# openhumanoids/pronto

Hardware: AMD Instinct MI355X
Metric: EKF predict+update steps/sec (batched filters), 15-state, 1000 Hz IMU (higher is better)
Workload: dtype f64

## Files before the change

### pronto_amd/csrc/pb_ctx.hpp

```cpp
#pragma once

#include <hip/hip_runtime.h>

#include <algorithm>
#include <cstdarg>
#include <cstdio>
#include <cstdlib>
#include <cstring>
#include <type_traits>
#include <vector>

#include "../../include/pronto_batch.h"
#include "rbis_tile_io.hpp"
#include "rbis_coop.hpp"
#include "rbis_legodo.hpp"
#include "rbis_jointfilt.hpp"
#include "rbis_yawlock.hpp"
#include "rbis_score.hpp"

using namespace pb;

#define PB_MAX_FENCES 16

struct pb_ctx {
// ... 41 lines not shown
  uint8_t *yaw_standing = nullptr;
  double *yaw_gyro = nullptr;
  bool yaw_standing_dev = false, yaw_gyro_dev = false;
  int yaw_standing_all = 0;
  double yaw_gyro_all = 0.0;
  ScorePar score_par;
  double *scored = nullptr;
  int64_t *scorei = nullptr;
  double *notch = nullptr;
  NotchCoef notch_coef;
  bool notch_ready = false;
  double *ins_last = nullptr;
  int64_t *ins_prev_ut = nullptr;
  const uint8_t *imu_valid_next = nullptr;
  const uint8_t *imu_valid_cur = nullptr;
  double *imu_keep = nullptr;
  const uint8_t *imu_idle_cur = nullptr;
  hipEvent_t fence[PB_MAX_FENCES] = {};
  int n_fences = 0;
  hipEvent_t ev_upload = nullptr;
  void *stage = nullptr;
  size_t stage_bytes = 0;
  void *in_stage[2] = { nullptr, nullptr };
  size_t in_stage_bytes[2] = { 0, 0 };
  int in_idx = 0;
  hipStream_t copy_stream = nullptr;
  hipEvent_t ev_consumed[2] = { nullptr, nullptr }, ev_copied = nullptr;
  Consts k{ 9.80665, 1e-6 };
  int64_t utime = 0;
  bool have_state = false;
  bool half15 = false;
  bool replay_onelane = false;
  bool coop15 = false;
  int mem_hint = 0;
  int run_block = 0, run_block_hint = 0;
  bool run_block_coop15 = false;
  bool quad21 = true;
  bool generic_update = false;
  bool smooth_attr = false;
  bool smooth_wide_attr = false;
  int n_cu = 256;
  hipEvent_t ev0 = nullptr, ev1 = nullptr;
  std::vector<void *> owned;
  char err[512] = { 0 };
};

inline thread_local char g_create_err[512] = "";

inline int fail(pb_ctx *c, int code, const char *fmt, ...)
{
  char *dst = c ? c->err : g_create_err;
  va_list ap;
  va_start(ap, fmt);
  vsnprintf(dst, 512, fmt, ap);
  va_end(ap);
  return code;
}

#define HIPCHK(c, call)                                                                               \
  do {                                                                                                \
    hipError_t e_ = (call);                                                                           \
    if (e_ != hipSuccess) return fail((c), PB_ERR_HIP, "%s failed: %s", #call, hipGetErrorString(e_)); \
  } while (0)

inline int nblk(int n) { return (n + 63) / 64; }

// ... 122 lines not shown
    }
    if (what & LEG_TIMES) {
      if (c->leg_ut_on) times.utimes = c->leg_ut_ext ? c->leg_ut_ext : c->leg_ut;
      if (c->leg_valid_on) times.valid = c->leg_valid_ext ? c->leg_valid_ext : c->leg_valid;
      c->leg_ut_on = c->leg_valid_on = false;
      c->leg_ut_ext = nullptr;
      c->leg_valid_ext = nullptr;
    }
    HIPCHK(c, hipSetDevice(c->dev));
    if ((what & (PRED_REFUSE | PRED_FORGET)) && c->pred_slot >= 0) {
      c->pred_slot = -1;
      if (what & PRED_REFUSE)
        return fail(c, PB_ERR_STATE, "%s: no predicted slot here (pb_set_pred_slot is for pb_step_legodo / _split / _correct)", fn);
    }
    if ((what & PRED_WITH_OUT) && c->pred_slot >= 0 && c->out_slot < 0) {
      c->pred_slot = -1;
      return fail(c, PB_ERR_STATE, "%s: no predicted slot here without an output slot (pb_set_output_slot)", fn);
    }
    if ((what & NEEDS_STATE) && !c->have_state) return fail(c, PB_ERR_STATE, "%s before pb_reset", fn);
    if ((what & PRED_TAKE) && c->pred_slot >= 0 && (c->pred_slot >= c->nhist || c->pred_slot == c->out_slot || c->pred_slot == pb_head_slot(c)))
      return fail(c, PB_ERR_ARG, "predicted slot %d: out of range, the output slot or the head's slot", c->pred_slot);
    return PB_OK;
  }
};
#define CALL(c, flags)               \
  Call call((c), __func__, (flags)); \
  if (call.rc) return call.rc

const double *pbk_idle_prepare(pb_ctx *c, const double *imu_dev, StepBcast &bc, int *rc_out);
int pbk_idle_restore(pb_ctx *c, double *out, double *pred, const double q[4]);

int pbk_step(pb_ctx *c, bool update, const double *imu, const double *lo, const uint8_t *mask, const double q[4],
             const StepBcast *bcast = nullptr);
int pbk_step_range(pb_ctx *c, const double *imu, const double *lo, const uint8_t *mask, const double q[4], long b0, int nb, bool coop15, int mem_hint);
int pbk_step_leg(pb_ctx *c, const double *imu, const StepBcast *bcast, const double q[4], const LegIn &lin, int64_t utime, const LegMeasPar &mp,
                 double *lo_out, uint8_t *mask_out);
int pbk_step_leg15(pb_ctx *c, double *out, const double *imu, const double q[4], const StepBcast &bc, const LegIn &lin, const LegStepArgs &la);
int pbk_step_leg21(pb_ctx *c, double *out, const double *imu, const double q[4], const StepBcast &bc, const LegIn &lin, const LegStepArgs &la);
int pbk_legpar15(pb_ctx *c, double *out, const double *imu, const double q[4], const StepBcast &bc, const LegIn &lin, const LegStepArgs &la);
int pbk_legpar21(pb_ctx *c, double *out, const double *imu, const double q[4], const StepBcast &bc, const LegIn &lin, const LegStepArgs &la);
int pbk_replay_fused(pb_ctx *c, int T, const double *imu, const double *lo, const uint8_t *mask, const double q[4], int slot0 = -1);
int pbk_step_pred_kernel(pb_ctx *c, double *out, double *pred, const double *imu, const double *lo, const uint8_t *mask, const double q[4],
                         const StepBcast &bc);
int pbk_step_corr_pred_kernel(pb_ctx *c, int corr_kind, double *out, double *pred, const double *imu, const double *lo, const uint8_t *mask,
                              const double q[4], const CorrArgs &ca, const StepBcast &bc);
int pbk_step_correct(pb_ctx *c, int corr_kind, const double *imu, const double *lo, const uint8_t *mask, const double q[4],
                     const double *z2, const double *r2, const double *rb2, const double *qm2, const uint8_t *mask2,
                     const StepBcast *bcast = nullptr, const double *zb = nullptr, const double *qb = nullptr);
int pbk_update15(pb_ctx *c, int m, const int *idx, const double *z, const double *R, int rkind, const double *rb,
                 const double *qm, const uint8_t *mask);
int pbk_update21(pb_ctx *c, int m, const int *idx, const double *z, const double *R, int rkind, const double *rb,
                 const double *qm, const uint8_t *mask);
int pbk_update21_m123(pb_ctx *c, int m, const int *idx, const double *z, const double *R, int rkind, const double *rb, const double *qm,
                      const uint8_t *mask);
int pbk_update21_m45(pb_ctx *c, int m, const int *idx, const double *z, const double *R, int rkind, const double *rb, const double *qm,
                     const uint8_t *mask);
int pbk_update21_m6(pb_ctx *c, int m, const int *idx, const double *z, const double *R, int rkind, const double *rb, const double *qm,
                    const uint8_t *mask);
int pbk_update_ct(pb_ctx *c, int m, const int *idx, const double *z, const double *r2, const double *rb2, const double *qm,
                  const uint8_t *mask, const double *zb = nullptr, const double *qb = nullptr, const double *rfull = nullptr);
int pbk_smooth_step(pb_ctx *c, const double *next_pred, const double *next_sm, const double *cur, double *out, double dt);
int pbk_smooth_wide(pb_ctx *c, const double *next_pred, const double *next_sm, const double *cur, double *out, double dt);
int pbk_slot_select(pb_ctx *c, double *dst, const double *src, const uint8_t *mask_dev, int when);
int pbk_update_common(pb_ctx *c, int m, const int *idx, const double *z, const double *R, int rkind, const double *qm, bool orient,
                      const uint8_t *mask, int mem);
```

### pronto_amd/csrc/pb_step.hip

```cpp
#include "pb_ctx.hpp"
#include "rbis_step_kernels.hpp"
#include "rbis_replay_kernels.hpp"

template <bool UPDATE, int MH>
static void launch_step_kernel(pb_ctx *c, const double *st, double *out, int nb, bool coop15, bool half, const double *imu, const double *lo,
                               const uint8_t *mask, const double q[4], const StepBcast &bc, const Consts &k)
{
  const int B = c->B;
  if (c->ns == 15 && coop15) {
    Consts kk = k;
    kk.half_tiles = half ? 1 : 0;
    k_step_coop<15, UPDATE, MH><<<nblk(nb) * (half ? 2 : 1), 128, 0, c->stream>>>(st, out, B, imu, lo, mask, q[0], q[1], q[2], q[3], kk, CorrArgs(), bc);
  } else if (c->ns == 15) {
    k_step<15, UPDATE, MH><<<(nb + PB_STEP_BLOCK - 1) / PB_STEP_BLOCK, PB_STEP_BLOCK, 0, c->stream>>>(st, out, B, imu, lo, mask, q[0], q[1], q[2], q[3], k, bc);
  } else if (c->quad21) {
    k_step_quad<UPDATE, MH><<<nblk(nb), 256, 0, c->stream>>>(st, out, B, imu, lo, mask, q[0], q[1], q[2], q[3], k, bc);
  } else {
    k_step_coop<21, UPDATE, MH><<<nblk(nb), 128, 0, c->stream>>>(st, out, B, imu, lo, mask, q[0], q[1], q[2], q[3], k, CorrArgs(), bc);
  }
}

template <bool UPDATE>
static int launch_step(pb_ctx *c, const double *imu, const double *lo, const uint8_t *mask, const double q[4], const StepBcast &bcast)
{
  double *out = update_target(c);
  int rc = PB_OK;
  StepBcast bc = bcast;
  imu = pbk_idle_prepare(c, imu, bc, &rc);
  if (rc) return rc;
  with_mem_hint(c->mem_hint, [&](auto mh) {
    launch_step_kernel<UPDATE, decltype(mh)::value>(c, c->st, out, c->B, c->coop15, c->half15, imu, lo, mask, q, bc, c->k);
  });
  LAUNCHCHK(c);
  if ((rc = pbk_idle_restore(c, out, nullptr, q))) return rc;
  update_done(c, out);
  return PB_OK;
}

int pbk_step_range(pb_ctx *c, const double *imu, const double *lo, const uint8_t *mask, const double q[4], long b0, int nb, bool coop15, int mem_hint)
{
  if (c->st != c->st_base || c->out_slot >= 0 || (c->B & 63) || (b0 & 63) || (nb & 63) || b0 + nb > c->B)
    return fail(c, PB_ERR_STATE, "pbk_step_range: whole tiles of a head that lives in the context's own array");
  const size_t tile_doubles = c->state_doubles / (size_t) (c->stride / 64);
  double *st = c->st + (size_t) (b0 / 64) * tile_doubles;
  const uint8_t *mask_b = mask ? mask + b0 : nullptr;
  Consts kk = c->k;
  if (kk.qblk) kk.qblk += b0;
  with_mem_hint(mem_hint, [&](auto mh) {
    launch_step_kernel<true, decltype(mh)::value>(c, st, st, nb, coop15, false, imu + b0, lo + b0, mask_b, q, StepBcast(), kk);
  });
  LAUNCHCHK(c);
  return PB_OK;
}

static int step_pred(pb_ctx *c, const double *imu, const double *lo, const uint8_t *mask, const double q[4], const StepBcast &bcast)
{
  double *pred = slot_ptr(c, c->pred_slot);
  const int ps = c->pred_slot;
  c->pred_slot = -1;
  int rc = PB_OK;
  StepBcast bc = bcast;
  imu = pbk_idle_prepare(c, imu, bc, &rc);
  if (rc) return rc;
  double *out = update_target(c);
  if (pbk_step_pred_kernel(c, out, pred, imu, lo, mask, q, bc) == PB_OK) {
    LAUNCHCHK(c);
    if ((rc = pbk_idle_restore(c, out, pred, q))) return rc;
    update_done(c, out);
    return PB_OK;
  }
  double *head = c->st;
  const int os = c->out_slot;
  c->out_slot = ps;
  rc = launch_step<false>(c, imu, nullptr, nullptr, q, bc);
  c->st = head;
  c->out_slot = os;
  if (rc) return rc;
  return launch_step<true>(c, imu, lo, mask, q, bc);
}

int pbk_step(pb_ctx *c, bool update, const double *imu, const double *lo, const uint8_t *mask, const double q[4],
             const StepBcast *bcast)
// ... 100 lines not shown
```

### pronto_amd/csrc/pronto_batch.hip

```cpp
#include <algorithm>
#include <new>

#include "pb_ctx.hpp"
#include "rbis_util_kernels.hpp"

#define PB_VERSION_STR "pronto_batch 0.3 gfx950"

extern "C" const char *pb_version(void) { return PB_VERSION_STR; }

extern "C" const char *pb_last_error(const pb_ctx *ctx) { return ctx ? ctx->err : g_create_err; }

extern "C" int pb_create(pb_ctx **out, int n_states, int batch, int device, int n_snapshots)
{
  if (!out) return fail(nullptr, PB_ERR_ARG, "pb_create: out is NULL");
  *out = nullptr;
  if (n_states != 15 && n_states != 21) return fail(nullptr, PB_ERR_ARG, "pb_create: n_states must be 15 or 21");
  if (batch <= 0 || n_snapshots < 0) return fail(nullptr, PB_ERR_ARG, "pb_create: bad batch / n_snapshots");
  int ndev = 0;
  if (hipGetDeviceCount(&ndev) != hipSuccess || ndev <= 0)
    return fail(nullptr, PB_ERR_NO_DEVICE, "pb_create: no HIP device visible (this library has no CPU fallback)");
  if (device < 0 || device >= ndev) return fail(nullptr, PB_ERR_ARG, "pb_create: device %d out of range", device);
  hipDeviceProp_t prop;
  HIPCHK(nullptr, hipGetDeviceProperties(&prop, device));
  if (strncmp(prop.gcnArchName, "gfx950", 6) != 0)
    return fail(nullptr, PB_ERR_NO_DEVICE, "pb_create: device %d is %s; kernels are built for gfx950 only", device,
                prop.gcnArchName);
  pb_ctx *c = new (std::nothrow) pb_ctx();
  if (!c) return fail(nullptr, PB_ERR_ARG, "pb_create: out of host memory");
  c->ns = n_states;
  c->B = batch;
  c->dev = device;
  c->nsnap = n_snapshots;
  c->n_cu = prop.multiProcessorCount > 0 ? prop.multiProcessorCount : 256;
  {
    const char *e = getenv("PRONTO_BATCH_COOP15");
    c->coop15 = e ? (e[0] == '1') : (batch <= 393216);
    const char *eh = getenv("PRONTO_BATCH_HALF");
    c->half15 = c->coop15 && n_states == 15 && eh && eh[0] == '1';
    const char *er = getenv("PRONTO_BATCH_REPLAY_ONELANE");
    c->replay_onelane = er && er[0] == '1';
  }
  c->stride = ((long) batch + 63) / 64 * 64;
  c->nc = (n_states == 15) ? Lay<15>::NC : Lay<21>::NC;
  c->state_doubles = (size_t) c->stride * (size_t) ((n_states == 15) ? Slots<15>::NSLOT : Slots<21>::NSLOT);
  {
    const char *e = getenv("PRONTO_BATCH_XCD");
    c->k.xcd_remap = e ? (e[0] == '1') : 1;
    const long state_bytes = (long) c->state_doubles * 8;
    const char *gu = getenv("PRONTO_BATCH_GENERIC_UPDATE");
    c->generic_update = gu && gu[0] == '1';
    const char *q21 = getenv("PRONTO_BATCH_QUAD21");
    c->quad21 = !(q21 && q21[0] == '0');
    const char *h = getenv("PRONTO_BATCH_MEMHINT");
    c->mem_hint = h ? (h[0] - '0')
                    : (state_bytes < (48L << 20)    ? MH_DEFAULT
                       : state_bytes < (310L << 20) ? MH_STORE_SC1
                       : state_bytes < (350L << 20) ? MH_DEFAULT
                                                    : MH_STREAM_NT);
    if (c->mem_hint < 0 || c->mem_hint > 2) c->mem_hint = MH_DEFAULT;
    {
      const char *eb = getenv("PRONTO_BATCH_BLOCKED"), *ef = getenv("PRONTO_BATCH_BLOCK_FILTERS");
      const long per_filter = state_bytes / c->stride;
      long want = ef ? atol(ef) : (n_states == 15 ? 229376 : 114688);
      want = (want + 63) / 64 * 64;
      const bool on = eb ? (eb[0] == '1') : (state_bytes > (256L << 20));
      if (on && want >= 64 && want < batch && (batch & 63) == 0) {
        const long nblocks = (batch + want - 1) / want;
        c->run_block = (int) (((batch + nblocks - 1) / nblocks + 63) / 64 * 64);
        const long blk_bytes = (long) c->run_block * per_filter;
        c->run_block_hint = h ? c->mem_hint : (blk_bytes < (48L << 20) ? MH_DEFAULT : MH_STORE_SC1);
        const char *e15 = getenv("PRONTO_BATCH_COOP15");
        c->run_block_coop15 = e15 ? (e15[0] == '1') : true;
      }
    }
  }
  if ((unsigned long long) batch * 36ull * 8ull >= (1ull << 32)) {
    delete c;
    return fail(nullptr, PB_ERR_ARG, "pb_create: batch %d too large for one context (input blocks must stay below 4 GiB; "
                "split the batch over several contexts)", batch);
  }
#define CRCHK(call) CRCHK_AS(#call, call)
#define CRCHK_AS(what, call)                                                                        \
  do {                                                                                              \
    hipError_t e_ = (call);                                                                         \
    if (e_ != hipSuccess) {                                                                         \
      fail(nullptr, PB_ERR_HIP, "%s failed: %s", what, hipGetErrorString(e_));                       \
      pb_destroy(c);                                                                                \
      return PB_ERR_HIP;                                                                            \
    }                                                                                               \
  } while (0)
  CRCHK(hipSetDevice(device));
  CRCHK(hipStreamCreateWithFlags(&c->own_stream, hipStreamNonBlocking));
  c->stream = c->own_stream;
  CRCHK_AS("hipMalloc (state)", dev_alloc_hip(c, c->st_base, c->state_doubles));
  c->st = c->st_base;
  CRCHK(hipMemsetAsync(c->st, 0, sizeof(double) * c->state_doubles, c->stream));
  if (n_snapshots > 0) {
    CRCHK_AS("hipMalloc (snapshots)", dev_alloc_hip(c, c->snaps, (size_t) 7 * c->stride * n_snapshots));
    CRCHK(hipMemsetAsync(c->snaps, 0, sizeof(double) * 7 * c->stride * n_snapshots, c->stream));
  }
  CRCHK_AS("hipMalloc (small staging)", dev_alloc_hip(c, c->d_small, 1024));
  CRCHK(hipEventCreate(&c->ev0));
  CRCHK(hipEventCreate(&c->ev1));
  CRCHK(hipStreamCreateWithFlags(&c->copy_stream, hipStreamNonBlocking));
  CRCHK(hipEventCreateWithFlags(&c->ev_consumed[0], hipEventDisableTiming));
// ... 39 lines not shown
{
  if (!c) return PB_ERR_ARG;
  if (c->stream != c->own_stream) HIPCHK(c, hipStreamSynchronize(c->stream));
  c->stream = c->own_stream;
  return PB_OK;
}

extern "C" int pb_set_constants(pb_ctx *c, double g, double chi_tol)
{
  if (!c) return PB_ERR_ARG;
  if (!(g > 0) || !(chi_tol >= 0)) return fail(c, PB_ERR_ARG, "pb_set_constants: g must be > 0 and chi_tol >= 0");
  c->k.g = g;
  c->k.chi_tol = chi_tol;
  return PB_OK;
}

extern "C" int pb_sync(pb_ctx *c)
{
  if (!c) return PB_ERR_ARG;
  HIPCHK(c, hipSetDevice(c->dev));
  HIPCHK(c, hipStreamSynchronize(c->stream));
  return PB_OK;
}

extern "C" int pb_run_block(const pb_ctx *c) { return c ? c->run_block : 0; }

extern "C" const char *pb_hot_kernel(const pb_ctx *c)
{
  if (!c) return "";
  static const char *const names[4][3] = { { "k_step_quad<true,0>", "k_step_quad<true,1>", "k_step_quad<true,2>" },
                                           { "k_step_coop<21,true,0>", "k_step_coop<21,true,1>", "k_step_coop<21,true,2>" },
                                           { "k_step_coop<15,true,0>", "k_step_coop<15,true,1>", "k_step_coop<15,true,2>" },
                                           { "k_step<15,true,0>", "k_step<15,true,1>", "k_step<15,true,2>" } };
  return names[c->ns == 21 ? (c->quad21 ? 0 : 1) : (c->coop15 ? 2 : 3)][c->mem_hint];
}
extern "C" int pb_batch(const pb_ctx *c) { return c ? c->B : -1; }
extern "C" int pb_n_states(const pb_ctx *c) { return c ? c->ns : -1; }

extern "C" int pb_malloc(pb_ctx *c, uint64_t bytes, void **p)
{
  if (!c || !p) return PB_ERR_ARG;
  HIPCHK(c, hipSetDevice(c->dev));
  HIPCHK(c, hipMalloc(p, bytes));
  return PB_OK;
}
extern "C" int pb_free(pb_ctx *c, void *p)
{
  if (!c) return PB_ERR_ARG;
  HIPCHK(c, hipSetDevice(c->dev));
  HIPCHK(c, hipStreamSynchronize(c->stream));
  HIPCHK(c, hipFree(p));
  return PB_OK;
}
extern "C" int pb_memcpy_h2d(pb_ctx *c, void *d, const void *h, uint64_t bytes)
{
  if (!c || (!d && bytes) || (!h && bytes)) return PB_ERR_ARG;
  HIPCHK(c, hipSetDevice(c->dev));
  HIPCHK(c, hipMemcpyAsync(d, h, bytes, hipMemcpyHostToDevice, c->stream));
  HIPCHK(c, hipStreamSynchronize(c->stream));
  return PB_OK;
}
extern "C" int pb_memcpy_d2h(pb_ctx *c, void *h, const void *d, uint64_t bytes)
{
  if (!c || (!d && bytes) || (!h && bytes)) return PB_ERR_ARG;
  HIPCHK(c, hipSetDevice(c->dev));
  HIPCHK(c, hipMemcpyAsync(h, d, bytes, hipMemcpyDeviceToHost, c->stream));
// ... 271 lines not shown
                { z2, sizeof(double) * m2 * B, 0 }, { rbc ? nullptr : R2, rbc ? 0 : sizeof(double) * m2 * B, 0 },
                { quat_meas2, sizeof(double) * 4 * B, 0 }, { mask2, B, 0 } };
  if (mem == PB_HOST_BROADCAST && mem2 == PB_HOST_BROADCAST && rbc && !mask && !mask2 && arg_kernel) {
    StepBcast bc;
    (void) imu_in(c, imu_block, mem, bc, p);
    memcpy(bc.lo, lo_block, sizeof(bc.lo));
    bc.on |= 2;
    return pbk_step_correct(c, corr_kind, nullptr, nullptr, nullptr, q, nullptr, nullptr, R2, nullptr, nullptr, &bc, z2, quat_meas2);
  }
  int rc;
  if (mem == mem2) rc = stage_in(c, mem, p, 7);
  else {
    rc = stage_in(c, mem, p, 3);
    if (!rc) rc = stage_in(c, mem2, p + 3, 4);
  }
  if (rc) return rc;
  return pbk_step_correct(c, corr_kind, (const double *) p[0].dev, (const double *) p[1].dev, (const uint8_t *) p[2].dev, q,
                          (const double *) p[3].dev, (const double *) p[4].dev, rbc ? R2 : nullptr, (const double *) p[5].dev,
                          (const uint8_t *) p[6].dev);
}

extern "C" int pb_run_legodo(pb_ctx *c, int n_steps, const double *imu_stream, const double *lo_stream,
                             const uint8_t *mask_stream, const double q[4], float *elapsed_ms)
{
  CALL(c, PRED_REFUSE | NEEDS_STATE);
  if (n_steps < 0 || !imu_stream || !lo_stream || !q) return fail(c, PB_ERR_ARG, "pb_run_legodo: bad argument");
  const size_t B = (size_t) c->B;
  if (int rc = timed_begin(c, elapsed_ms)) return rc;
  if (c->run_block > 0 && n_steps > 1 && c->st == c->st_base && c->out_slot < 0) {
    for (long b0 = 0; b0 < (long) B; b0 += c->run_block) {
      const int nb = (int) std::min<long>(c->run_block, (long) B - b0);
      for (int s = 0; s < n_steps; s++) {
        int rc = pbk_step_range(c, imu_stream + (size_t) s * 7 * B, lo_stream + (size_t) s * 6 * B,
                                mask_stream ? mask_stream + (size_t) s * B : nullptr, q, b0, nb, c->run_block_coop15, c->run_block_hint);
        if (rc) return rc;
      }
    }
  } else {
    for (int s = 0; s < n_steps; s++) {
      int rc = pbk_step(c, true, imu_stream + (size_t) s * 7 * B, lo_stream + (size_t) s * 6 * B,
                        mask_stream ? mask_stream + (size_t) s * B : nullptr, q);
      if (rc) return rc;
    }
  }
  return timed_end(c, elapsed_ms);
}

static int replay_impl(pb_ctx *c, const char *who, int n_steps, int steps_per_launch, const double *imu_stream, const double *lo_stream,
                       const uint8_t *mask_stream, const double q[4], bool write_through, int first_slot, float *elapsed_ms)
{
  if (n_steps < 0 || steps_per_launch < 1 || !imu_stream || !lo_stream || !q) return fail(c, PB_ERR_ARG, "%s: bad argument", who);
  if (write_through && (first_slot < 0 || first_slot + n_steps > c->nhist))
    return fail(c, PB_ERR_ARG, "%s: slots %d..%d of %d (pb_history_reserve)", who, first_slot, first_slot + n_steps - 1, c->nhist);
  const size_t B = (size_t) c->B;
  if (int rc = detach_head(c, true)) return rc;
  if (int rc = timed_begin(c, elapsed_ms)) return rc;
  for (int s = 0; s < n_steps; s += steps_per_launch) {
    const int T = (n_steps - s < steps_per_launch) ? n_steps - s : steps_per_launch;
    int rc = pbk_replay_fused(c, T, imu_stream + (size_t) s * 7 * B, lo_stream + (size_t) s * 6 * B,
                              mask_stream ? mask_stream + (size_t) s * B : nullptr, q, write_through ? first_slot + s : -1);
    if (rc) return rc;
  }
  return timed_end(c, elapsed_ms);
}

extern "C" int pb_replay_legodo_fused(pb_ctx *c, int n_steps, int steps_per_launch, const double *imu_stream,
                                      const double *lo_stream, const uint8_t *mask_stream, const double q[4],
// ... 382 lines not shown
```

### pronto_amd/csrc/rbis_device.hpp

```cpp
#pragma once

#include <cmath>
#include <type_traits>
#include <utility>

#if defined(__HIPCC__)
#include <hip/hip_runtime.h>
#define PB_HD __host__ __device__ __forceinline__
#else
#define PB_HD inline
#endif

namespace pb {

template <int NS>
struct Lay {
  static constexpr int NB = NS / 3;
  static constexpr int NP = NS * (NS + 1) / 2;
  static constexpr int OFF_VEC = 0;
  static constexpr int OFF_QUAT = NS;
  static constexpr int OFF_LL = NS + 4;
  static constexpr int OFF_P = NS + 5;
  static constexpr int NC = NS + 5 + NP;
};
// ... 9 lines not shown
  return i;
}
PB_HD constexpr int pk_col(int p) { return p - pk_row(p) * (pk_row(p) + 1) / 2; }

template <class Fn, int... I>
PB_HD void static_for_impl(Fn &&fn, std::integer_sequence<int, I...>)
{
  (fn(std::integral_constant<int, I>{}), ...);
}
template <int N, class Fn>
PB_HD void static_for(Fn &&fn)
{
  static_for_impl(fn, std::make_integer_sequence<int, N>{});
}

PB_HD constexpr int core_full(int s) { return s < 9 ? 3 + s : 15 + (s - 9); }
PB_HD constexpr int passive_full(int p) { return p < 3 ? p : 12 + (p - 3); }

template <int NS>
struct Slots {
  using L = Lay<NS>;
  static constexpr bool HB = (NS == 21);
  static constexpr int NSC = HB ? 15 : 9;
  static constexpr int NSB = HB ? 5 : 3;
  static constexpr int NROW = (L::NC + 1) / 2, NSLOT = 2 * NROW;
  static constexpr int TILE = 64;
  static constexpr long TILE_DOUBLES = (long) NSLOT * TILE;
  static constexpr unsigned TILE_BYTES = (unsigned) (NSLOT * TILE * 8);
  struct Tab {
    short slot_of[L::NC];
    short comp_of[NSLOT];
    signed char role2[NSLOT];
    bool split2[NROW];
    int ncore;
    int nq[4];
  };
  static constexpr Tab make()
  {
    Tab t{};
    int s = 0, role = 0;
    auto put = [&](int c) { t.slot_of[c] = (short) s; t.role2[s] = (signed char) role; t.comp_of[s++] = (short) c; };
    if (!HB) {
      for (int i = 0; i < 9; i++) put(L::OFF_VEC + 3 + i);
      for (int i = 0; i < 4; i++) put(L::OFF_QUAT + i);
      for (int i = 0; i < 9; i++)
        for (int j = 0; j <= i; j++) put(L::OFF_P + pk(core_full(i), core_full(j)));
      t.ncore = s;
      t.nq[0] = t.nq[1] = s;
      role = 1;
      for (int J = 0; J < 2; J++)
        for (int i = 0; i < NSC; i++)
          for (int cc = 0; cc < 3; cc++) put(L::OFF_P + pk(core_full(i), passive_full(3 * J + cc)));
      for (int i = 0; i < 6; i++)
        for (int j = 0; j <= i; j++) put(L::OFF_P + pk(passive_full(i), passive_full(j)));
      put(L::OFF_LL);
      for (int i = 0; i < 6; i++) put(L::OFF_VEC + passive_full(i));
      t.nq[2] = s;
    } else {
      for (int i = 0; i < 9; i++)
        for (int j = 0; j <= i; j++) put(L::OFF_P + pk(core_full(i), core_full(j)));
      put(L::OFF_LL);
      t.nq[0] = s;
      for (int i = 9; i < NSC; i++)
        for (int j = 0; j <= i; j++) put(L::OFF_P + pk(core_full(i), core_full(j)));
      for (int i = 0; i < 6; i++) put(L::OFF_VEC + 15 + i);
      role = 1;
      for (int i = 0; i < 3; i++) put(L::OFF_VEC + passive_full(i));
      t.nq[1] = s;
      t.ncore = s;
      for (int i = 0; i < NSC; i++)
        for (int cc = 0; cc < 3; cc++) put(L::OFF_P + pk(core_full(i), passive_full(cc)));
      for (int i = 0; i < 3; i++)
        for (int j = 0; j <= i; j++) put(L::OFF_P + pk(passive_full(i), passive_full(j)));
      role = 0;
      for (int i = 0; i < 9; i++) put(L::OFF_VEC + 3 + i);
      for (int i = 0; i < 4; i++) put(L::OFF_QUAT + i);
      t.nq[2] = s;
      role = 1;
      for (int i = 0; i < NSC; i++)
        for (int cc = 0; cc < 3; cc++) put(L::OFF_P + pk(core_full(i), passive_full(3 + cc)));
      for (int i = 3; i < 6; i++)
        for (int j = 0; j <= i; j++) put(L::OFF_P + pk(passive_full(i), passive_full(j)));
      for (int i = 3; i < 6; i++) put(L::OFF_VEC + passive_full(i));
    }
    while (s < NSLOT) { t.role2[s] = (signed char) role; t.comp_of[s++] = -1; }
    t.nq[3] = s;
    for (int r = 0; r < NROW; r++) t.split2[r] = t.role2[2 * r] != t.role2[2 * r + 1];
    return t;
  }
  static constexpr Tab T = make();
  static_assert(T.nq[0] % 2 == 0 && T.nq[1] % 2 == 0 && T.nq[2] % 2 == 0, "every wave must own whole rows");
  static constexpr int ROW_SPLIT = T.ncore / 2;
  static constexpr int QROW[5] = { 0, T.nq[0] / 2, T.nq[1] / 2, T.nq[2] / 2, T.nq[3] / 2 };
  PB_HD static constexpr int slot(int comp) { return T.slot_of[comp]; }
  PB_HD static long eidx(int comp, long b)
  {
    const int sl = T.slot_of[comp];
    return (b >> 6) * TILE_DOUBLES + (long) (sl >> 1) * (2 * TILE) + (b & 63) * 2 + (sl & 1);
  }
  PB_HD static long eidx_slot(int sl, long b) { return (b >> 6) * TILE_DOUBLES + (long) (sl >> 1) * (2 * TILE) + (b & 63) * 2 + (sl & 1); }
};

enum { BW = 0, BV = 1, BCHI = 2, BPOS = 3, BACC = 4, BBG = 5, BBA = 6 };

struct Consts {
  double g;
  double chi_tol;
  const double *qblk = nullptr;
  int xcd_remap = 0;
  int half_tiles = 0;
};

PB_HD void quat_mul(const double (&a)[4], const double (&b)[4], double (&o)[4])
{
  const double w = a[0] * b[0] - a[1] * b[1] - a[2] * b[2] - a[3] * b[3];
  const double x = a[0] * b[1] + a[1] * b[0] + a[2] * b[3] - a[3] * b[2];
  const double y = a[0] * b[2] + a[2] * b[0] + a[3] * b[1] - a[1] * b[3];
  const double z = a[0] * b[3] + a[3] * b[0] + a[1] * b[2] - a[2] * b[1];
  o[0] = w; o[1] = x; o[2] = y; o[3] = z;
}
// ... 440 lines not shown
```

### pronto_amd/csrc/rbis_step_kernels.hpp

```cpp
#pragma once

#include "rbis_tile_io.hpp"
#include "rbis_coop.hpp"
#include "rbis_quad.hpp"

namespace pb {

template <int NS, bool UPDATE, int MH = MH_DEFAULT>
__global__ __launch_bounds__(PB_STEP_BLOCK, 1) void k_step(const double *st, double *sto, int B,
                                                const double *__restrict__ imu, const double *__restrict__ lo,
                                                const uint8_t *__restrict__ mask, double qg, double qa, double qbg,
                                                double qba, Consts k, StepBcast bc)
{
  using L = Lay<NS>;
  const unsigned tile = xcd_workgroup(k);
  const unsigned b = tile * 64u + threadIdx.x;
  if (b >= (unsigned) B) return;
  const unsigned bo = b * 8u, B8 = (unsigned) B * 8u;
  TileIO<NS, MemHint<MH>::LA, MemHint<MH>::SA> io(st, sto, tile, threadIdx.x);
  const rsrc_t ri = mkbuf(imu, 7u * B8);
  const rsrc_t rl = mkbuf(lo, UPDATE ? 6u * B8 : 0u);
  double gyro[3], accel[3], dt, z[3], rd[3];
  bool upd = false;
  if constexpr (UPDATE) upd = (mask == nullptr) || (mask[b] != 0);
  if (bc.on & 1) {
#pragma unroll
    for (int i = 0; i < 3; i++) { gyro[i] = bc.imu[i]; accel[i] = bc.imu[3 + i]; }
    dt = bc.imu[6];
  } else {
#pragma unroll
    for (int i = 0; i < 3; i++) {
      gyro[i] = ldg(ri, i * B8, bo);
      accel[i] = ldg(ri, (3 + i) * B8, bo);
    }
    dt = ldg(ri, 6u * B8, bo);
  }
// ... 93 lines not shown
    const rsrc_t rr = mkbuf(ca.r2, ca.r2 ? (unsigned) CORR::M * B8 : 0u);
    const rsrc_t rq2 = mkbuf(ca.qm2, CORR::ORIENT ? 4u * B8 : 0u);
#pragma unroll
    for (int i = 0; i < CORR::M; i++) {
      cin.z[i] = ca.zbc ? ca.zb2[i] : ldg(rz, i * B8, bo);
      cin.rd[i] = ca.r2 ? ldg(rr, i * B8, bo) : ca.rb2[i];
    }
    if (ca.rfull != nullptr) {
      const rsrc_t rf = mkbuf(ca.rfull, (unsigned) (CORR::M * CORR::M) * B8);
#pragma unroll
      for (int i = 0; i < CORR::M; i++) {
        cin.rd[i] = ldg(rf, (unsigned) (i * CORR::M + i) * B8, bo);
#pragma unroll
        for (int j = 0; j < i; j++) cin.ro[i * (i - 1) / 2 + j] = ldg(rf, (unsigned) (j * CORR::M + i) * B8, bo);
      }
    }
#pragma unroll
    for (int i = 0; i < 4; i++) cin.qm[i] = CORR::ORIENT ? (ca.zbc ? ca.qb2[i] : ldg(rq2, i * B8, bo)) : 0.0;
    cin.upd = (b < (unsigned) B) && (ca.mask2 == nullptr || ca.mask2[b] != 0);
    if constexpr (!PREDICT && !UPDATE) {
      if (st == sto && ca.mask2 != nullptr && __ballot(cin.upd) == 0ull) return;
    }
  }
  auto ld = [&io](int comp) { return io.ld(comp); };
  auto stf = [&io](int comp, double v) { io.st(comp, v); };
  auto sync = []() { __syncthreads(); };
  auto xrd = [lane](int s) { return xch[s][lane]; };
  if (role == 0) {
    io.template need<0, Slots<NS>::ROW_SPLIT>();
    coop_role_core<NS, UPDATE, CORR, PREDICT>(ld, stf, [lane](int s, double v) { xch[s][lane] = v; }, xrd, sync, in, k, cin);
  } else {
    io.template need<Slots<NS>::ROW_SPLIT, Slots<NS>::NROW>();
    coop_role_passive<NS, UPDATE, CORR, PREDICT>(ld, stf, xrd, sync, in, k, cin);
  }
}

template <class IO>
struct PredStore {
  static constexpr bool on = true;
  IO *io;
  __device__ __forceinline__ void operator()(int comp, double v) const { io->st(comp, v); }
};

template <int NS, int MH = MH_DEFAULT>
__global__ __launch_bounds__(128, 1) void k_step_coop_pred(const double *st, double *sto, double *pred, int B,
                                                           const double *__restrict__ imu, const double *__restrict__ lo,
                                                           const uint8_t *__restrict__ mask, double qg, double qa,
                                                           double qbg, double qba, Consts k, StepBcast bc)
{
  __shared__ double xch[CoopX<NS, NoCorr>::NXCH][64];
  const int role = __builtin_amdgcn_readfirstlane((int) (threadIdx.x >> 6));
  const unsigned wgi = xcd_workgroup(k);
  const unsigned tile = k.half_tiles ? (wgi >> 1) : wgi;
  const unsigned lane = k.half_tiles ? ((threadIdx.x & 31u) | ((wgi & 1u) << 5)) : (threadIdx.x & 63u);
  const unsigned b = tile * 64u + lane;
  const unsigned bo = b * 8u, B8 = (unsigned) B * 8u;
  using IO = TileIO<NS, MemHint<MH>::LA, MemHint<MH>::SA, true>;
  IO io(st, sto, tile, lane);
  IO po(pred, pred, tile, lane);
  const rsrc_t ri = mkbuf(imu, 7u * B8);
  const rsrc_t rl = mkbuf(lo, 6u * B8);
  StepInputs in;
  if (bc.on & 1) {
#pragma unroll
    for (int i = 0; i < 3; i++) { in.gyro[i] = bc.imu[i]; in.accel[i] = bc.imu[3 + i]; }
    in.dt = bc.imu[6];
// ... 252 lines not shown
```

### pronto_amd/csrc/rbis_tile_io.hpp

```cpp
#pragma once

#include <hip/hip_runtime.h>
#include <stdint.h>

#include "rbis_device.hpp"

#define PB_STEP_BLOCK 64

namespace pb {

typedef unsigned v2u __attribute__((ext_vector_type(2)));
typedef unsigned v4u __attribute__((ext_vector_type(4)));
typedef double d2_t __attribute__((ext_vector_type(2)));
typedef __amdgpu_buffer_rsrc_t rsrc_t;

__device__ __forceinline__ rsrc_t mkbuf(const void *p, unsigned bytes)
{
  return __builtin_amdgcn_make_buffer_rsrc(const_cast<void *>(p), 0, bytes, 0x00020000);
}
template <int AUX = 0>
__device__ __forceinline__ double ldg(rsrc_t r, unsigned soff, unsigned voff)
{
  return __builtin_bit_cast(double, __builtin_amdgcn_raw_buffer_load_b64(r, voff, soff, AUX));
}
// ... 1 lines not shown
__device__ __forceinline__ void stg(rsrc_t r, unsigned soff, unsigned voff, double v)
{
  __builtin_amdgcn_raw_buffer_store_b64(__builtin_bit_cast(v2u, v), r, voff, soff, AUX);
}
template <int AUX = 0>
__device__ __forceinline__ d2_t ldg2(rsrc_t r, unsigned soff, unsigned voff)
{
  return __builtin_bit_cast(d2_t, __builtin_amdgcn_raw_buffer_load_b128(r, voff, soff, AUX));
}
template <int AUX = 0>
__device__ __forceinline__ void stg2(rsrc_t r, unsigned soff, unsigned voff, d2_t v)
{
  const v4u d = __builtin_bit_cast(v4u, v);
  __builtin_amdgcn_raw_buffer_store_b128(d, r, voff, soff, AUX);
  asm volatile("s_nop 1" ::"v"(d));
}

enum { MH_DEFAULT = 0, MH_STORE_SC1 = 1, MH_STREAM_NT = 2 };
template <int MH> struct MemHint {
  static constexpr int LA = (MH == MH_STREAM_NT) ? 2 : 0;
  static constexpr int SA = (MH == MH_STORE_SC1) ? 16 : (MH == MH_STREAM_NT) ? 2 : 0;
};

__device__ __forceinline__ unsigned xcd_workgroup(const Consts &k)
{
  unsigned wg = blockIdx.x;
  if (k.xcd_remap) {
    const unsigned nq = gridDim.x >> 3, nr = gridDim.x & 7u, xcd = blockIdx.x & 7u, rank = blockIdx.x >> 3;
    wg = (xcd < nr ? xcd * (nq + 1u) : nr * (nq + 1u) + (xcd - nr) * nq) + rank;
  }
  return wg;
}

template <int NS, int LA, int SA, bool TWO_ROLE = false>
struct TileIO {
  using S = Slots<NS>;
  rsrc_t rs, ro;
  unsigned vo;
  d2_t cache[S::NROW];
  bool loaded[S::NROW];
  double outv[S::NSLOT];
  bool have[S::NSLOT];
  __device__ __forceinline__ TileIO(const double *st, double *sto, unsigned tile, unsigned lane)
  {
    rs = mkbuf(reinterpret_cast<const char *>(st) + (size_t) tile * S::TILE_BYTES, S::TILE_BYTES);
    ro = mkbuf(reinterpret_cast<char *>(sto) + (size_t) tile * S::TILE_BYTES, S::TILE_BYTES);
    vo = lane * 16u;
#pragma unroll
    for (int r = 0; r < S::NROW; r++) loaded[r] = false;
#pragma unroll
    for (int s = 0; s < S::NSLOT; s++) {
      have[s] = S::T.comp_of[s] < 0;
      outv[s] = 0.0;
    }
  }
  __device__ __forceinline__ void fetch(int r)
  {
    if (!loaded[r]) {
      cache[r] = ldg2<LA>(rs, (unsigned) r * 1024u, vo);
      loaded[r] = true;
    }
  }
  template <int R0, int R1>
  __device__ __forceinline__ void need()
  {
#pragma unroll
    for (int r = R0; r < R1; r++) fetch(r);
  }
  __device__ __forceinline__ double ld(int comp)
  {
    const int s = S::T.slot_of[comp];
    fetch(s >> 1);
    return (s & 1) ? cache[s >> 1].y : cache[s >> 1].x;
  }
  __device__ __forceinline__ void st(int comp, double v)
  {
    const int s = S::T.slot_of[comp];
    if (TWO_ROLE && S::T.split2[s >> 1]) {
      stg<SA>(ro, (unsigned) (s >> 1) * 1024u + (unsigned) (s & 1) * 8u, vo, v);
      return;
    }
    outv[s] = v;
    have[s] = true;
    if (have[s ^ 1]) {
      const d2_t o = { outv[s & ~1], outv[s | 1] };
      stg2<SA>(ro, (unsigned) (s >> 1) * 1024u, vo, o);
    }
  }
  __device__ __forceinline__ double ld_slot_rt(int slot) const
  {
    return ldg(rs, (unsigned) (slot >> 1) * 1024u + (unsigned) (slot & 1) * 8u, vo);
  }
};

template <int NS>
__device__ __forceinline__ int slot_rt(int comp)
{
  return Slots<NS>::T.slot_of[comp];
}
__device__ __forceinline__ int pk_rt(int i, int j) { return i >= j ? i * (i + 1) / 2 + j : j * (j + 1) / 2 + i; }

struct IdxVel {
  static constexpr Idx<3> value = { { 3, 4, 5 } };
};

template <int M>
struct IdxArg {
  int v[M];
};
template <int M>
struct DiagArg {
// ... 31 lines not shown
```

Measured before the change: 2.756 billion.

## Add balanced two-role 15-state step kernel splitting covariance work between wavefronts

Adds k_step_bal15, a two-wavefront cooperative kernel for the 15-state filter. One wave owns the 9x9 core covariance block and computes the 3x3 innovation factorization and gain rows. The other wave propagates the cross and bias blocks plus the state, exchanging values through LDS with one barrier. The aim is to balance work between the two roles better than the existing coop kernel. It is enabled by default only for specific batch-size ranges and adds a new store-split table, which costs extra code complexity and LDS traffic.

```diff
diff --git a/pronto_amd/csrc/pb_ctx.hpp b/pronto_amd/csrc/pb_ctx.hpp
--- a/pronto_amd/csrc/pb_ctx.hpp
+++ b/pronto_amd/csrc/pb_ctx.hpp
@@ -97,6 +97,7 @@
   bool half15 = false;
   bool replay_onelane = false;
   bool coop15 = false;
+  bool bal15 = false, run_block_bal15 = false;
   int mem_hint = 0;
   int run_block = 0, run_block_hint = 0;
   bool run_block_coop15 = false;
@@ -285,7 +286,8 @@
 
 int pbk_step(pb_ctx *c, bool update, const double *imu, const double *lo, const uint8_t *mask, const double q[4],
              const StepBcast *bcast = nullptr);
-int pbk_step_range(pb_ctx *c, const double *imu, const double *lo, const uint8_t *mask, const double q[4], long b0, int nb, bool coop15, int mem_hint);
+int pbk_step_range(pb_ctx *c, const double *imu, const double *lo, const uint8_t *mask, const double q[4], long b0, int nb, bool coop15, bool bal15,
+                   int mem_hint);
 int pbk_step_leg(pb_ctx *c, const double *imu, const StepBcast *bcast, const double q[4], const LegIn &lin, int64_t utime, const LegMeasPar &mp,
                  double *lo_out, uint8_t *mask_out);
 int pbk_step_leg15(pb_ctx *c, double *out, const double *imu, const double q[4], const StepBcast &bc, const LegIn &lin, const LegStepArgs &la);
diff --git a/pronto_amd/csrc/pb_step.hip b/pronto_amd/csrc/pb_step.hip
--- a/pronto_amd/csrc/pb_step.hip
+++ b/pronto_amd/csrc/pb_step.hip
@@ -3,11 +3,13 @@
 #include "rbis_replay_kernels.hpp"
 
 template <bool UPDATE, int MH>
-static void launch_step_kernel(pb_ctx *c, const double *st, double *out, int nb, bool coop15, bool half, const double *imu, const double *lo,
+static void launch_step_kernel(pb_ctx *c, const double *st, double *out, int nb, bool coop15, bool half, bool bal15, const double *imu, const double *lo,
                                const uint8_t *mask, const double q[4], const StepBcast &bc, const Consts &k)
 {
   const int B = c->B;
-  if (c->ns == 15 && coop15) {
+  if (UPDATE && c->ns == 15 && coop15 && bal15 && !half) {
+    k_step_bal15<true, MH><<<nblk(nb), 128, 0, c->stream>>>(st, out, B, imu, lo, mask, q[0], q[1], q[2], q[3], k, bc);
+  } else if (c->ns == 15 && coop15) {
     Consts kk = k;
     kk.half_tiles = half ? 1 : 0;
     k_step_coop<15, UPDATE, MH><<<nblk(nb) * (half ? 2 : 1), 128, 0, c->stream>>>(st, out, B, imu, lo, mask, q[0], q[1], q[2], q[3], kk, CorrArgs(), bc);
@@ -29,7 +31,7 @@
   imu = pbk_idle_prepare(c, imu, bc, &rc);
   if (rc) return rc;
   with_mem_hint(c->mem_hint, [&](auto mh) {
-    launch_step_kernel<UPDATE, decltype(mh)::value>(c, c->st, out, c->B, c->coop15, c->half15, imu, lo, mask, q, bc, c->k);
+    launch_step_kernel<UPDATE, decltype(mh)::value>(c, c->st, out, c->B, c->coop15, c->half15, c->bal15, imu, lo, mask, q, bc, c->k);
   });
   LAUNCHCHK(c);
   if ((rc = pbk_idle_restore(c, out, nullptr, q))) return rc;
@@ -37,7 +39,8 @@
   return PB_OK;
 }
 
-int pbk_step_range(pb_ctx *c, const double *imu, const double *lo, const uint8_t *mask, const double q[4], long b0, int nb, bool coop15, int mem_hint)
+int pbk_step_range(pb_ctx *c, const double *imu, const double *lo, const uint8_t *mask, const double q[4], long b0, int nb, bool coop15, bool bal15,
+                   int mem_hint)
 {
   if (c->st != c->st_base || c->out_slot >= 0 || (c->B & 63) || (b0 & 63) || (nb & 63) || b0 + nb > c->B)
     return fail(c, PB_ERR_STATE, "pbk_step_range: whole tiles of a head that lives in the context's own array");
@@ -47,7 +50,7 @@
   Consts kk = c->k;
   if (kk.qblk) kk.qblk += b0;
   with_mem_hint(mem_hint, [&](auto mh) {
-    launch_step_kernel<true, decltype(mh)::value>(c, st, st, nb, coop15, false, imu + b0, lo + b0, mask_b, q, StepBcast(), kk);
+    launch_step_kernel<true, decltype(mh)::value>(c, st, st, nb, coop15, false, bal15, imu + b0, lo + b0, mask_b, q, StepBcast(), kk);
   });
   LAUNCHCHK(c);
   return PB_OK;
diff --git a/pronto_amd/csrc/pronto_batch.hip b/pronto_amd/csrc/pronto_batch.hip
--- a/pronto_amd/csrc/pronto_batch.hip
+++ b/pronto_amd/csrc/pronto_batch.hip
@@ -9,6 +9,8 @@
 extern "C" const char *pb_version(void) { return PB_VERSION_STR; }
 
 extern "C" const char *pb_last_error(const pb_ctx *ctx) { return ctx ? ctx->err : g_create_err; }
+
+static bool bal15_default(long n) { return (n >= 32768 && n <= 49152) || (n >= 98304 && n <= 131072) || n == 393216; }
 
 extern "C" int pb_create(pb_ctx **out, int n_states, int batch, int device, int n_snapshots)
 {
@@ -37,6 +39,8 @@
     c->coop15 = e ? (e[0] == '1') : (batch <= 393216);
     const char *eh = getenv("PRONTO_BATCH_HALF");
     c->half15 = c->coop15 && n_states == 15 && eh && eh[0] == '1';
+    const char *eb = getenv("PRONTO_BATCH_BAL15");
+    c->bal15 = n_states == 15 && c->coop15 && !c->half15 && (eb ? (eb[0] == '1') : bal15_default(batch));
     const char *er = getenv("PRONTO_BATCH_REPLAY_ONELANE");
     c->replay_onelane = er && er[0] == '1';
   }
@@ -71,6 +75,8 @@
         c->run_block_hint = h ? c->mem_hint : (blk_bytes < (48L << 20) ? MH_DEFAULT : MH_STORE_SC1);
         const char *e15 = getenv("PRONTO_BATCH_COOP15");
         c->run_block_coop15 = e15 ? (e15[0] == '1') : true;
+        const char *eb15 = getenv("PRONTO_BATCH_BAL15");
+        c->run_block_bal15 = n_states == 15 && c->run_block_coop15 && (eb15 ? (eb15[0] == '1') : bal15_default(c->run_block));
       }
     }
   }
@@ -176,6 +182,8 @@
                                            { "k_step_coop<21,true,0>", "k_step_coop<21,true,1>", "k_step_coop<21,true,2>" },
                                            { "k_step_coop<15,true,0>", "k_step_coop<15,true,1>", "k_step_coop<15,true,2>" },
                                            { "k_step<15,true,0>", "k_step<15,true,1>", "k_step<15,true,2>" } };
+  static const char *const bal[3] = { "k_step_bal15<true,0>", "k_step_bal15<true,1>", "k_step_bal15<true,2>" };
+  if (c->ns == 15 && c->coop15 && c->bal15) return bal[c->mem_hint];
   return names[c->ns == 21 ? (c->quad21 ? 0 : 1) : (c->coop15 ? 2 : 3)][c->mem_hint];
 }
 extern "C" int pb_batch(const pb_ctx *c) { return c ? c->B : -1; }
@@ -513,7 +521,8 @@
       const int nb = (int) std::min<long>(c->run_block, (long) B - b0);
       for (int s = 0; s < n_steps; s++) {
         int rc = pbk_step_range(c, imu_stream + (size_t) s * 7 * B, lo_stream + (size_t) s * 6 * B,
-                                mask_stream ? mask_stream + (size_t) s * B : nullptr, q, b0, nb, c->run_block_coop15, c->run_block_hint);
+                                mask_stream ? mask_stream + (size_t) s * B : nullptr, q, b0, nb, c->run_block_coop15, c->run_block_bal15,
+                                c->run_block_hint);
         if (rc) return rc;
       }
     }
diff --git a/pronto_amd/csrc/rbis_coop_bal.hpp b/pronto_amd/csrc/rbis_coop_bal.hpp
--- /dev/null
+++ b/pronto_amd/csrc/rbis_coop_bal.hpp
@@ -0,0 +1,290 @@
+#pragma once
+
+#include "rbis_coop.hpp"
+
+namespace pb {
+
+struct Bal15 {
+  static constexpr int NS = 15, NSC = 9, NPC = 45;
+  static constexpr int X_L = 0, X_ID = 3, X_W = 6, X_NL = 6 + 3 * NSC;
+  static constexpr int NXCH = X_NL + 1;
+};
+
+template <bool UPDATE, class LD, class ST, class XW, class SYNC>
+PB_HD void bal15_role_core(LD ld, ST st, XW xw, SYNC sync, const StepInputs &in, const Consts &k)
+{
+  constexpr int NS = Bal15::NS, NSC = Bal15::NSC;
+  using L = Lay<NS>;
+  using C = Coop<NS>;
+  double x[NS], q[4];
+#pragma unroll
+  for (int i = 0; i < NS; i++) x[i] = ld(L::OFF_VEC + i);
+#pragma unroll
+  for (int i = 0; i < 4; i++) q[i] = ld(L::OFF_QUAT + i);
+  double Pc[Bal15::NPC];
+#pragma unroll
+  for (int i = 0; i < NSC; i++)
+#pragma unroll
+    for (int j = 0; j <= i; j++) Pc[pk(i, j)] = ld(L::OFF_P + pk(C::fullc(i), C::fullc(j)));
+
+  ProcBlocks f;
+  make_proc_blocks<NS>(x, q, in.dt, k, f);
+  if constexpr (!UPDATE) sync();
+  {
+    const int src[2] = { 0, 1 };
+    const int kind[2] = { 0, 0 };
+    double A[2][9];
+#pragma unroll
+    for (int i = 0; i < 9; i++) { A[0][i] = f.A_R[i]; A[1][i] = f.A_RV[i]; }
+    RowOp<NSC, 2, 2>::apply(Pc, src, kind, A);
+  }
+  {
+    const int src[2] = { 0, 1 };
+    const int kind[2] = { 1, 1 };
+    double A[2][9];
+#pragma unroll
+    for (int i = 0; i < 9; i++) { A[0][i] = f.a_mw[i % 3]; A[1][i] = f.a_g[i % 3]; }
+    RowOp<NSC, 0, 2>::apply(Pc, src, kind, A);
+    const int src2[1] = { 1 };
+    const int kind2[1] = { 1 };
+    double A2[1][9];
+#pragma unroll
+    for (int i = 0; i < 9; i++) A2[0][i] = f.a_mw[i % 3];
+    RowOp<NSC, 1, 1>::apply(Pc, src2, kind2, A2);
+  }
+  {
+    const double qgd = in.qg * in.dt, qad = in.qa * in.dt;
+    const double vv = f.v[0] * f.v[0] + f.v[1] * f.v[1] + f.v[2] * f.v[2];
+#pragma unroll
+    for (int r = 0; r < 3; r++)
+#pragma unroll
+      for (int c = 0; c <= r; c++) Pc[pk(r, c)] += qgd * ((r == c ? vv : 0.0) - f.v[r] * f.v[c]) + (r == c ? qad : 0.0);
+    const double m[9] = { 0, f.v[2], -f.v[1], -f.v[2], 0, f.v[0], f.v[1], -f.v[0], 0 };
+#pragma unroll
+    for (int r = 0; r < 3; r++)
+#pragma unroll
+      for (int c = 0; c < 3; c++)
+        if (r != c) Pc[pk(3 + r, c)] += qgd * m[3 * r + c];
+#pragma unroll
+    for (int r = 0; r < 3; r++) Pc[pk(3 + r, 3 + r)] += qgd;
+  }
+  if constexpr (!UPDATE) {
+#pragma unroll
+    for (int i = 0; i < NSC; i++)
+#pragma unroll
+      for (int j = 0; j <= i; j++) st(L::OFF_P + pk(C::fullc(i), C::fullc(j)), Pc[pk(i, j)]);
+  } else {
+    double S[6], d[3], id[3];
+#pragma unroll
+    for (int i = 0; i < 3; i++)
+#pragma unroll
+      for (int j = 0; j <= i; j++) S[pk(i, j)] = Pc[pk(i, j)] + (i == j ? (in.upd ? in.rd[i] : 1.0) : 0.0);
+    ldlt<3>(S, d);
+    double det = 1.0;
+#pragma unroll
+    for (int kk = 0; kk < 3; kk++) {
+      id[kk] = in.upd ? 1.0 / d[kk] : 0.0;
+      det *= d[kk];
+    }
+    const double nl = -log(det);
+    double W[NSC][3];
+#pragma unroll
+    for (int i = 0; i < NSC; i++)
+#pragma unroll
+      for (int kk = 0; kk < 3; kk++) {
+        double s = Pc[pk(i, kk)];
+#pragma unroll
+        for (int j = 0; j < kk; j++) s -= W[i][j] * S[pk(kk, j)];
+        W[i][kk] = s;
+      }
+    xw(Bal15::X_L, S[pk(1, 0)]); xw(Bal15::X_L + 1, S[pk(2, 0)]); xw(Bal15::X_L + 2, S[pk(2, 1)]);
+#pragma unroll
+    for (int kk = 0; kk < 3; kk++) xw(Bal15::X_ID + kk, id[kk]);
+#pragma unroll
+    for (int i = 0; i < NSC; i++)
+#pragma unroll
+      for (int kk = 0; kk < 3; kk++) xw(Bal15::X_W + 3 * i + kk, W[i][kk]);
+    xw(Bal15::X_NL, nl);
+    sync();
+#pragma unroll
+    for (int i = 0; i < NSC; i++) {
+      double wd[3];
+#pragma unroll
+      for (int kk = 0; kk < 3; kk++) wd[kk] = W[i][kk] * id[kk];
+#pragma unroll
+      for (int j = 0; j <= i; j++) {
+        double acc = Pc[pk(i, j)];
+#pragma unroll
+        for (int kk = 0; kk < 3; kk++) acc = fma(-wd[kk], W[j][kk], acc);
+        st(L::OFF_P + pk(C::fullc(i), C::fullc(j)), acc);
+      }
+    }
+  }
+}
+
+template <bool UPDATE, class LD, class ST, class XR, class SYNC>
+PB_HD void bal15_role_passive(LD ld, ST st, XR xr, SYNC sync, const StepInputs &in, const Consts &k)
+{
+  constexpr int NS = Bal15::NS, NSC = Bal15::NSC;
+  using L = Lay<NS>;
+  using C = Coop<NS>;
+  double x[NS], q[4];
+#pragma unroll
+  for (int i = 0; i < NS; i++) x[i] = ld(L::OFF_VEC + i);
+#pragma unroll
+  for (int i = 0; i < 4; i++) q[i] = ld(L::OFF_QUAT + i);
+  double X[3][2][9];
+#pragma unroll
+  for (int sb = 0; sb < 3; sb++)
+#pragma unroll
+    for (int J = 0; J < 2; J++)
+#pragma unroll
+      for (int r = 0; r < 3; r++)
+#pragma unroll
+        for (int c = 0; c < 3; c++) X[sb][J][3 * r + c] = ld(L::OFF_P + pk(C::fullc(3 * sb + r), C::fullp(3 * J + c)));
+  double Ppp[21];
+#pragma unroll
+  for (int i = 0; i < 6; i++)
+#pragma unroll
+    for (int j = 0; j <= i; j++) Ppp[pk(i, j)] = ld(L::OFF_P + pk(C::fullp(i), C::fullp(j)));
+  double ll = ld(L::OFF_LL);
+
+  double xp[6];
+  {
+    ProcBlocks f;
+    make_proc_blocks<NS>(x, q, in.dt, k, f);
+#pragma unroll
+    for (int J = 0; J < 2; J++) {
+      double nD[9], nV[9], nC[9];
+#pragma unroll
+      for (int i = 0; i < 9; i++) { nD[i] = X[2][J][i]; nV[i] = X[0][J][i]; nC[i] = X[1][J][i]; }
+      mat_mul_acc(f.A_R, X[0][J], nD);
+      mat_mul_acc(f.A_RV, X[1][J], nD);
+      hat_mul_acc(f.a_mw, X[0][J], nV);
+      hat_mul_acc(f.a_g, X[1][J], nV);
+      hat_mul_acc(f.a_mw, X[1][J], nC);
+#pragma unroll
+      for (int i = 0; i < 9; i++) { X[2][J][i] = nD[i]; X[0][J][i] = nV[i]; X[1][J][i] = nC[i]; }
+    }
+  }
+#pragma unroll
+  for (int r = 0; r < 3; r++)
+#pragma unroll
+    for (int c = 0; c <= r; c++) {
+      Ppp[pk(r, c)] = (r == c) ? in.qg : 0.0;
+      Ppp[pk(3 + r, 3 + c)] = (r == c) ? in.qa : 0.0;
+    }
+#pragma unroll
+  for (int i = 0; i < 3; i++) {
+    xp[i] = in.gyro[i] - 0.0;
+    xp[3 + i] = in.accel[i] - 0.0;
+  }
+#pragma unroll
+  for (int i = 0; i < 4; i++) pb_pin(q[i]);
+#pragma unroll
+  for (int sb = 0; sb < 3; sb++)
+#pragma unroll
+    for (int J = 0; J < 2; J++)
+#pragma unroll
+      for (int i = 0; i < 9; i++) pb_pin(X[sb][J][i]);
+#pragma unroll
+  for (int i = 0; i < 9; i++) pb_pin(x[C::fullc(i)]);
+  ins_update_state<NS>(x, q, in.gyro, in.accel, in.dt, k);
+#pragma unroll
+  for (int i = 0; i < 9; i++) pb_pin(x[C::fullc(i)]);
+#pragma unroll
+  for (int i = 0; i < 4; i++) pb_pin(q[i]);
+  sync();
+  if constexpr (UPDATE) {
+    const double L10 = xr(Bal15::X_L), L20 = xr(Bal15::X_L + 1), L21 = xr(Bal15::X_L + 2);
+    const double Ls[6] = { 0.0, L10, 0.0, L20, L21, 0.0 };
+    double id[3], resid[3], y[3], yd[3];
+#pragma unroll
+    for (int kk = 0; kk < 3; kk++) id[kk] = xr(Bal15::X_ID + kk);
+#pragma unroll
+    for (int i = 0; i < 3; i++) resid[i] = in.upd ? in.z[i] - x[3 + i] : 0.0;
+    double quad = 0.0;
+#pragma unroll
+    for (int kk = 0; kk < 3; kk++) {
+      double s = resid[kk];
+#pragma unroll
+      for (int j = 0; j < kk; j++) s -= Ls[pk(kk, j)] * y[j];
+      y[kk] = in.upd ? s : 0.0;
+      yd[kk] = y[kk] * id[kk];
+      quad += s * s * id[kk];
+    }
+    const double lli = xr(Bal15::X_NL) - quad;
+    if (in.upd) ll += lli;
+    double Wp[6][3];
+#pragma unroll
+    for (int pi = 0; pi < 6; pi++) {
+      const double c0 = X[0][pi / 3][0 * 3 + pi % 3], c1 = X[0][pi / 3][1 * 3 + pi % 3], c2 = X[0][pi / 3][2 * 3 + pi % 3];
+      Wp[pi][0] = c0;
+      Wp[pi][1] = c1 - Wp[pi][0] * L10;
+      Wp[pi][2] = c2 - Wp[pi][0] * L20 - Wp[pi][1] * L21;
+      xp[pi] += fma(Wp[pi][2], yd[2], fma(Wp[pi][1], yd[1], Wp[pi][0] * yd[0]));
+    }
+#pragma unroll
+    for (int J = 0; J < 2; J++)
+#pragma unroll
+      for (int sb = 0; sb < 3; sb++)
+#pragma unroll
+        for (int r = 0; r < 3; r++) {
+          double wd[3];
+#pragma unroll
+          for (int kk = 0; kk < 3; kk++) wd[kk] = xr(Bal15::X_W + 3 * (3 * sb + r) + kk) * id[kk];
+#pragma unroll
+          for (int c = 0; c < 3; c++) {
+            double acc = X[sb][J][3 * r + c];
+#pragma unroll
+            for (int kk = 0; kk < 3; kk++) acc = fma(-wd[kk], Wp[3 * J + c][kk], acc);
+            st(L::OFF_P + pk(C::fullc(3 * sb + r), C::fullp(3 * J + c)), acc);
+          }
+        }
+#pragma unroll
+    for (int i = 0; i < 6; i++) {
+      double wd[3];
+#pragma unroll
+      for (int kk = 0; kk < 3; kk++) wd[kk] = Wp[i][kk] * id[kk];
+#pragma unroll
+      for (int j = 0; j <= i; j++) {
+        double acc = Ppp[pk(i, j)];
+#pragma unroll
+        for (int kk = 0; kk < 3; kk++) acc = fma(-wd[kk], Wp[j][kk], acc);
+        st(L::OFF_P + pk(C::fullp(i), C::fullp(j)), acc);
+      }
+    }
+    reload_fence();
+    double dfull[NS];
+#pragma unroll
+    for (int i = 0; i < NS; i++) dfull[i] = 0.0;
+#pragma unroll
+    for (int i = 0; i < NSC; i++) {
+      const double w0 = xr(Bal15::X_W + 3 * i), w1 = xr(Bal15::X_W + 3 * i + 1), w2 = xr(Bal15::X_W + 3 * i + 2);
+      dfull[C::fullc(i)] = fma(w2, yd[2], fma(w1, yd[1], w0 * yd[0])) + 0.0;
+    }
+    if (in.upd) add_delta<NS>(x, q, dfull, k.chi_tol);
+  } else {
+#pragma unroll
+    for (int J = 0; J < 2; J++)
+#pragma unroll
+      for (int sb = 0; sb < 3; sb++)
+#pragma unroll
+        for (int r = 0; r < 3; r++)
+#pragma unroll
+          for (int c = 0; c < 3; c++) st(L::OFF_P + pk(C::fullc(3 * sb + r), C::fullp(3 * J + c)), X[sb][J][3 * r + c]);
+#pragma unroll
+    for (int i = 0; i < 6; i++)
+#pragma unroll
+      for (int j = 0; j <= i; j++) st(L::OFF_P + pk(C::fullp(i), C::fullp(j)), Ppp[pk(i, j)]);
+  }
+  st(L::OFF_LL, ll);
+#pragma unroll
+  for (int i = 0; i < 6; i++) st(L::OFF_VEC + C::fullp(i), xp[i]);
+#pragma unroll
+  for (int i = 0; i < 9; i++) st(L::OFF_VEC + C::fullc(i), x[C::fullc(i)]);
+#pragma unroll
+  for (int i = 0; i < 4; i++) st(L::OFF_QUAT + i, q[i]);
+}
+
+}
diff --git a/pronto_amd/csrc/rbis_device.hpp b/pronto_amd/csrc/rbis_device.hpp
--- a/pronto_amd/csrc/rbis_device.hpp
+++ b/pronto_amd/csrc/rbis_device.hpp
@@ -65,6 +65,8 @@
     short comp_of[NSLOT];
     signed char role2[NSLOT];
     bool split2[NROW];
+    signed char role2b[NSLOT];
+    bool split2b[NROW];
     int ncore;
     int nq[4];
   };
@@ -119,6 +121,11 @@
     while (s < NSLOT) { t.role2[s] = (signed char) role; t.comp_of[s++] = -1; }
     t.nq[3] = s;
     for (int r = 0; r < NROW; r++) t.split2[r] = t.role2[2 * r] != t.role2[2 * r + 1];
+    for (int sl = 0; sl < NSLOT; sl++) {
+      const int c = t.comp_of[sl];
+      t.role2b[sl] = HB ? t.role2[sl] : (signed char) ((c >= L::OFF_P && sl < t.ncore) ? 0 : 1);
+    }
+    for (int r = 0; r < NROW; r++) t.split2b[r] = t.role2b[2 * r] != t.role2b[2 * r + 1];
     return t;
   }
   static constexpr Tab T = make();
diff --git a/pronto_amd/csrc/rbis_step_kernels.hpp b/pronto_amd/csrc/rbis_step_kernels.hpp
--- a/pronto_amd/csrc/rbis_step_kernels.hpp
+++ b/pronto_amd/csrc/rbis_step_kernels.hpp
@@ -2,6 +2,7 @@
 
 #include "rbis_tile_io.hpp"
 #include "rbis_coop.hpp"
+#include "rbis_coop_bal.hpp"
 #include "rbis_quad.hpp"
 
 namespace pb {
@@ -161,6 +162,68 @@
   } else {
     io.template need<Slots<NS>::ROW_SPLIT, Slots<NS>::NROW>();
     coop_role_passive<NS, UPDATE, CORR, PREDICT>(ld, stf, xrd, sync, in, k, cin);
+  }
+}
+
+template <bool UPDATE, int MH = MH_DEFAULT>
+__global__ __launch_bounds__(128, 1) void k_step_bal15(const double *st, double *sto, int B,
+                                                       const double *__restrict__ imu, const double *__restrict__ lo,
+                                                       const uint8_t *__restrict__ mask, double qg, double qa,
+                                                       double qbg, double qba, Consts k, StepBcast bc)
+{
+  constexpr int NS = 15;
+  __shared__ double xch[UPDATE ? Bal15::NXCH : 1][64];
+  const int role = __builtin_amdgcn_readfirstlane((int) (threadIdx.x >> 6));
+  const unsigned tile = xcd_workgroup(k);
+  const unsigned lane = threadIdx.x & 63u;
+  const unsigned b = tile * 64u + lane;
+  const unsigned bo = b * 8u, B8 = (unsigned) B * 8u;
+  TileIO<NS, MemHint<MH>::LA, MemHint<MH>::SA, 2> io(st, sto, tile, lane);
+  auto inputs = [&](bool core) {
+    const rsrc_t ri = mkbuf(imu, 7u * B8);
+    const rsrc_t rl = mkbuf(lo, UPDATE ? 6u * B8 : 0u);
+    StepInputs in;
+    if (bc.on & 1) {
+#pragma unroll
+      for (int i = 0; i < 3; i++) { in.gyro[i] = bc.imu[i]; in.accel[i] = bc.imu[3 + i]; }
+      in.dt = bc.imu[6];
+    } else {
+#pragma unroll
+      for (int i = 0; i < 3; i++) {
+        in.gyro[i] = core ? 0.0 : ldg(ri, i * B8, bo);
+        in.accel[i] = core ? 0.0 : ldg(ri, (3 + i) * B8, bo);
+      }
+      in.dt = ldg(ri, 6u * B8, bo);
+    }
+    if (bc.on & 2) {
+#pragma unroll
+      for (int i = 0; i < 3; i++) { in.z[i] = bc.lo[i]; in.rd[i] = bc.lo[3 + i]; }
+    } else {
+#pragma unroll
+      for (int i = 0; i < 3; i++) {
+        in.z[i] = (UPDATE && !core) ? ldg(rl, i * B8, bo) : 0.0;
+        in.rd[i] = (UPDATE && core) ? ldg(rl, (3 + i) * B8, bo) : 1.0;
+      }
+    }
+    in.upd = UPDATE && (b < (unsigned) B) && (mask == nullptr || mask[b] != 0);
+    in.qg = qg; in.qa = qa; in.qbg = qbg; in.qba = qba;
+    if (k.qblk != nullptr) {
+      const rsrc_t rq = mkbuf(k.qblk, 4u * B8);
+      in.qg = ldg(rq, 0u, bo); in.qa = ldg(rq, B8, bo); in.qbg = ldg(rq, 2u * B8, bo); in.qba = ldg(rq, 3u * B8, bo);
+    }
+    return in;
+  };
+  auto ld = [&io](int comp) { return io.ld(comp); };
+  auto stf = [&io](int comp, double v) { io.st(comp, v); };
+  auto sync = []() { __syncthreads(); };
+  if (role != 0) {
+    const StepInputs in = inputs(false);
+    io.template need<Slots<NS>::ROW_SPLIT, Slots<NS>::NROW>();
+    bal15_role_passive<UPDATE>(ld, stf, [lane](int s) { return xch[s][lane]; }, sync, in, k);
+  } else {
+    const StepInputs in = inputs(true);
+    io.template need<0, Slots<NS>::ROW_SPLIT>();
+    bal15_role_core<UPDATE>(ld, stf, [lane](int s, double v) { xch[s][lane] = v; }, sync, in, k);
   }
 }
 
diff --git a/pronto_amd/csrc/rbis_tile_io.hpp b/pronto_amd/csrc/rbis_tile_io.hpp
--- a/pronto_amd/csrc/rbis_tile_io.hpp
+++ b/pronto_amd/csrc/rbis_tile_io.hpp
@@ -57,7 +57,7 @@
   return wg;
 }
 
-template <int NS, int LA, int SA, bool TWO_ROLE = false>
+template <int NS, int LA, int SA, int TWO_ROLE = 0>
 struct TileIO {
   using S = Slots<NS>;
   rsrc_t rs, ro;
@@ -101,7 +101,7 @@
   __device__ __forceinline__ void st(int comp, double v)
   {
     const int s = S::T.slot_of[comp];
-    if (TWO_ROLE && S::T.split2[s >> 1]) {
+    if (TWO_ROLE != 0 && (TWO_ROLE == 2 ? S::T.split2b[s >> 1] : S::T.split2[s >> 1])) {
       stg<SA>(ro, (unsigned) (s >> 1) * 1024u + (unsigned) (s & 1) * 8u, vo, v);
       return;
     }
```

Result: slower. 2.712 billion (-1.6%).
